# jhidalgocarrio/slam-localization

Measured on NVIDIA B200. Metric: filter-steps/sec (predict+update), higher is better.
Workload: dtype f64

## Files before the change

slam-localization_b200/csrc/slb_usckf_step.cuh:

```cuda
#pragma once
#include "slb_predict12.cuh"

#ifndef SLB_USCKF_CTA_SYNC
#define SLB_USCKF_CTA_SYNC 0
#endif
#if SLB_USCKF_CTA_SYNC
#define SLB_CTA_SYNC() __syncthreads()
#else
#define SLB_CTA_SYNC() ((void)0)
#endif

namespace slbd {

template <int NK_, int NL_>
struct StepCfg {
    static constexpr int NK = NK_, NL = NL_, NF = NK_ + NL_;
    static constexpr int N = 36 + NK_ + NL_;
    static constexpr int NP = N * (N + 1) / 2;
    static constexpr int PSTR = (NP + 15) / 16 * 16;
    static constexpr int QD = 39 + NK_ + NL_;
    static constexpr int QS = (QD + 1) / 2 * 2;
    static constexpr int NT = (N + 7) / 8;
    static constexpr int NPAD = 8 * NT;
    static constexpr int JM = 36 + NK_;
    static constexpr int NPAN = (JM + 3) / 4;
    static constexpr int NCOL = 4 * NPAN;
    static constexpr int JLAST = (NCOL - 1) >> 3;
    static constexpr int NGRP = (NPAN + 3) / 4;
    static constexpr int PL = 2 * NPAD + 8;
    static constexpr int PS4 = 2 * PL + 2;
    static constexpr int KP = (NK_ + 3) / 4 * 4;
    static constexpr int LF = 4 * PS4;
    static constexpr int LRAW = 2 * PL;
    static constexpr int KK = 2 * NPAD * KP + NPAD;
    static constexpr int SCR0 = (LF + LRAW > KK ? LF + LRAW : KK);
    static constexpr int WGS = 16 * NK_;
    static constexpr int UPD_SCR = SCR0 + WGS + NPAD;
    static constexpr int PRED_SCR = PRED_LS + 28 * PRED_DS + 144 + 12 * PRED_DS + 16 + 16;
    static constexpr int SCR = (UPD_SCR > PRED_SCR ? UPD_SCR : PRED_SCR);
    static constexpr int ZS = (NK_ + 1) / 2 * 2;
    static constexpr int SM = PSTR + QS + SCR + ZS + 2;
    static_assert(NK_ % 3 == 0 && NK_ >= 3, "the VO model moves 3-D features");
    static_assert(N <= 64, "two rows per lane");
    static_assert(SM % 2 == 0 && PSTR % 2 == 0 && QS % 2 == 0, "16-byte alignment of the bulk copies");
};

SLB_DEV void bulk_s2g(void *gdst, const void *ssrc, unsigned bytes) {
    asm volatile("cp.async.bulk.global.shared::cta.bulk_group [%0], [%1], %2;\n cp.async.bulk.commit_group;\n" ::"l"(gdst),
                 "r"(saddr(ssrc)), "r"(bytes)
                 : "memory");
}
SLB_DEV void bulk_prefetch_l2(const void *gsrc, unsigned bytes) {
    asm volatile("cp.async.bulk.prefetch.L2.global [%0], %1;\n" ::"l"(gsrc), "r"(bytes) : "memory");
}
SLB_DEV void bulk_store_wait() { asm volatile("cp.async.bulk.wait_group.read 0;\n" ::: "memory"); }
SLB_DEV void fence_proxy_async() { asm volatile("fence.proxy.async.shared::cta;\n" ::: "memory"); }

template <int M>
SLB_DEV bool sym_inverse(const double *S, double *Si) {
    double L[M * (M + 1) / 2], dd[M], rd[M];
    bool ok = true;
#pragma unroll
    for (int k = 0; k < M; ++k) {
        double d = S[tri(k, k)];
#pragma unroll
        for (int p = 0; p < k; ++p) d = fma(-L[tri(k, p)] * L[tri(k, p)], dd[p], d);
        ok = ok && (d > 0.0);
        dd[k] = d;
        rd[k] = rcp_fast(d);
#pragma unroll
        for (int i = k + 1; i < M; ++i) {
            double s = S[tri(i, k)];
#pragma unroll
            for (int p = 0; p < k; ++p) s = fma(-L[tri(i, p)] * L[tri(k, p)], dd[p], s);
            L[tri(i, k)] = s * rd[k];
        }
    }
    double X[M * (M + 1) / 2];
#pragma unroll
    for (int j = 0; j < M; ++j) {
        X[tri(j, j)] = 1.0;
#pragma unroll
        for (int i = j + 1; i < M; ++i) {
            double s = 0.0;
#pragma unroll
            for (int p = j; p < i; ++p) s = fma(-L[tri(i, p)], X[tri(p, j)], s);
            X[tri(i, j)] = s;
        }
    }
#pragma unroll
    for (int i = 0; i < M; ++i)
#pragma unroll
        for (int j = 0; j <= i; ++j) {
            double s = 0.0;
#pragma unroll
            for (int k = i; k < M; ++k) s = fma(X[tri(k, i)] * rd[k], X[tri(k, j)], s);
            Si[tri(i, j)] = s;
        }
    return ok;
}

template <int NK>
SLB_DEV void vo_model(const double *pk, const double *qk, const double *pi, const double *qi, const double *f, double *z) {
    double dq[4];
    quat_cmul(qi, qk, dq);
#pragma unroll
    for (int c = 0; c < NK; c += 3) {
        double rz[3];
        rotmat_apply(dq, f + c, rz);
        z[c] = rz[0] + (pk[0] - pi[0]);
        z[c + 1] = rz[1] + (pk[1] - pi[1]);
        z[c + 2] = rz[2] + (pk[2] - pi[2]);
    }
}

SLB_DEV void warp_sum12(const double *v, double *out, double *slots, int lane) {
    double a[8], b[4], c[2], d1;
    const bool h16 = lane & 16, h8 = lane & 8, h4 = lane & 4, h2 = lane & 2;
#pragma unroll
    for (int i = 0; i < 8; ++i) {
        const double lo = v[i], hi = i < 4 ? v[8 + i] : 0.0;
        const double r = __shfl_xor_sync(FULL, h16 ? lo : hi, 16);
        a[i] = (h16 ? hi : lo) + r;
    }
#pragma unroll
    for (int i = 0; i < 4; ++i) {
        const double r = __shfl_xor_sync(FULL, h8 ? a[i] : a[4 + i], 8);
        b[i] = (h8 ? a[4 + i] : a[i]) + r;
    }
#pragma unroll
    for (int i = 0; i < 2; ++i) {
        const double r = __shfl_xor_sync(FULL, h4 ? b[i] : b[2 + i], 4);
        c[i] = (h4 ? b[2 + i] : b[i]) + r;
    }
    {
        const double r = __shfl_xor_sync(FULL, h2 ? c[0] : c[1], 2);
        d1 = (h2 ? c[1] : c[0]) + r;
    }
    d1 += __shfl_xor_sync(FULL, d1, 1);
    const int idx = (h16 ? 8 : 0) + (h8 ? 4 : 0) + (h4 ? 2 : 0) + (h2 ? 1 : 0);
    __syncwarp();
    if (!(lane & 1)) slots[idx] = d1;
    __syncwarp();
#pragma unroll
    for (int i = 0; i < 6; ++i) {
        const double2 t = *reinterpret_cast<const double2 *>(slots + 2 * i);
        out[2 * i] = t.x;
        out[2 * i + 1] = t.y;
    }
}

template <class C>
struct UpdState {
    double c0[C::NT][C::JLAST + 1], c1[C::NT][C::JLAST + 1];
    double px0[C::NK], px1[C::NK];
    double esum[C::NK], eep[C::NK * (C::NK + 1) / 2];
    double z0[C::NK];
    bool ok;
};

template <class C, int G>
SLB_DEV void sigma_group(UpdState<C> &s, const double *mus_, const double *Lf, double *Wg, const double *dv, int lane) {
    constexpr int NK = C::NK, PS4 = C::PS4;
    double mus[40 + NK];
    {
        const double2 *m2 = reinterpret_cast<const double2 *>(mus_);
#pragma unroll
        for (int e = 0; e < 4; ++e) { const double2 v = m2[e]; mus[2 * e] = v.x; mus[2 * e + 1] = v.y; }
#pragma unroll
        for (int e = 13; e < 17; ++e) { const double2 v = m2[e]; mus[2 * e] = v.x; mus[2 * e + 1] = v.y; }
#pragma unroll
        for (int c = 0; c < NK; ++c) mus[39 + c] = mus_[39 + c];
    }
    constexpr int col0 = 16 * G;
    constexpr int ncols = C::NCOL - col0 < 16 ? C::NCOL - col0 : 16;
    const bool neg = lane & 1, act = (lane >> 1) < ncols;
    const int jl = act ? lane >> 1 : 0;
    const double rs = rsqrt_fast(dv[col0 + jl]);
    const double sgn = act ? (neg ? -rs : rs) : 0.0;
    const double *col = Lf + (jl >> 2) * PS4 + ((jl & 3) >> 1) * C::PL + (jl & 1);
    auto Lc = [&](int r) -> double { return sgn * col[2 * r]; };
    double xpk[3], xqk[4], xpi[3], xqi[4], xf[NK];
    if (col0 <= 5) {
#pragma unroll
        for (int c = 0; c < 3; ++c) xpk[c] = mus[c] + Lc(c);
        const double v[3] = {Lc(3), Lc(4), Lc(5)};
        const double q[4] = {mus[3], mus[4], mus[5], mus[6]};
        double e[4];
        so3_exp(v, 1.0, e);
        quat_mul(q, e, xqk);
    } else {
#pragma unroll
        for (int c = 0; c < 3; ++c) xpk[c] = mus[c];
#pragma unroll
        for (int c = 0; c < 4; ++c) xqk[c] = mus[3 + c];
    }
    if (col0 <= 29) {
#pragma unroll
        for (int c = 0; c < 3; ++c) xpi[c] = mus[26 + c] + Lc(24 + c);
        const double v[3] = {Lc(27), Lc(28), Lc(29)};
        const double q[4] = {mus[29], mus[30], mus[31], mus[32]};
        double e[4];
        so3_exp(v, 1.0, e);
        quat_mul(q, e, xqi);
    } else {
#pragma unroll
        for (int c = 0; c < 3; ++c) xpi[c] = mus[26 + c];
#pragma unroll
        for (int c = 0; c < 4; ++c) xqi[c] = mus[29 + c];
    }
#pragma unroll
    for (int c = 0; c < NK; ++c) xf[c] = mus[39 + c] + Lc(36 + c);
    double z[NK];
    vo_model<NK>(xpk, xqk, xpi, xqi, xf, z);
    double e[NK];
#pragma unroll
    for (int c = 0; c < NK; ++c) {
        e[c] = act ? z[c] - s.z0[c] : 0.0;
        s.esum[c] += e[c];
        const double zp = __shfl_xor_sync(FULL, z[c], 1);
        if (act && !neg) Wg[c * 16 + jl] = (0.5 * rs) * (z[c] - zp);
    }
#pragma unroll
    for (int r = 0; r < NK; ++r)
#pragma unroll
        for (int c = 0; c <= r; ++c) s.eep[tri(r, c)] = fma(e[r], e[c], s.eep[tri(r, c)]);
    __syncwarp();
    const bool has1 = lane + 32 < C::NPAD;
#pragma unroll
    for (int qq = 0; qq < ncols / 4; ++qq) {
        const double *pa = Lf + qq * PS4 + 2 * lane, *pb = pa + C::PL;
        const double2 x01 = *reinterpret_cast<const double2 *>(pa), x23 = *reinterpret_cast<const double2 *>(pb);
        double2 y01 = make_double2(0.0, 0.0), y23 = y01;
        if (has1) { y01 = *reinterpret_cast<const double2 *>(pa + 64); y23 = *reinterpret_cast<const double2 *>(pb + 64); }
#pragma unroll
        for (int c = 0; c < NK; ++c) {
            const double2 w01 = *reinterpret_cast<const double2 *>(Wg + c * 16 + 4 * qq);
            const double2 w23 = *reinterpret_cast<const double2 *>(Wg + c * 16 + 4 * qq + 2);
            s.px0[c] = fma(x23.y, w23.y, fma(x23.x, w23.x, fma(x01.y, w01.y, fma(x01.x, w01.x, s.px0[c]))));
            s.px1[c] = fma(y23.y, w23.y, fma(y23.x, w23.x, fma(y01.y, w01.y, fma(y01.x, w01.x, s.px1[c]))));
        }
    }
}

template <class C, int P>
struct PanelStep {
    SLB_DEV static void run(UpdState<C> &s, const double *mus, double *Lf, double *Lraw, double *Wg, double *dv, int lane) {
        constexpr int NT = C::NT, JLAST = C::JLAST, PS4 = C::PS4;
        constexpr int K = 4 * P, J0 = K >> 3, H = (K >> 2) & 1, Q = P & 3;
        constexpr int I1 = (K + 4) >> 3;
        const int a_ = lane & 3, b_ = lane >> 2;
        double *Lq = Lf + Q * PS4;
        constexpr int PL = C::PL;
        if ((a_ >> 1) == H) {
#pragma unroll
            for (int I = J0; I < NT; ++I)
                *reinterpret_cast<double2 *>(Lraw + (a_ & 1) * PL + 2 * (8 * I + b_)) = make_double2(s.c0[I][J0], s.c1[I][J0]);
        }
        __syncwarp();
        double m10, m20, m30, m21, m31, m32, r0, r1, r2, r3, d0, d1, d2, d3;
        {
            const double *A = Lraw + 2 * K, *Bp = A + PL;
            const double a00 = A[0];
            const double2 a1 = *reinterpret_cast<const double2 *>(A + 2);
            const double2 a2 = *reinterpret_cast<const double2 *>(A + 4);
            const double a22 = Bp[4];
            const double2 a3 = *reinterpret_cast<const double2 *>(A + 6), a3b = *reinterpret_cast<const double2 *>(Bp + 6);
            d0 = a00;
            r0 = rcp_fast(d0);
            m10 = a1.x * r0; m20 = a2.x * r0; m30 = a3.x * r0;
            d1 = fma(-a1.x, m10, a1.y);
            const double u21 = fma(-a2.x, m10, a2.y), u31 = fma(-a3.x, m10, a3.y);
            r1 = rcp_fast(d1);
            m21 = u21 * r1; m31 = u31 * r1;
            d2 = fma(-u21, m21, fma(-a2.x, m20, a22));
            const double u32 = fma(-u31, m21, fma(-a3.x, m20, a3b.x));
            r2 = rcp_fast(d2);
            m32 = u32 * r2;
            d3 = fma(-u32, m32, fma(-u31, m31, fma(-a3.x, m30, a3b.y)));
            r3 = rcp_fast(d3);
            s.ok = s.ok && (d0 > 0.0) && (d1 > 0.0) && (d2 > 0.0) && (d3 > 0.0);
        }
        if (lane == 0) {
            *reinterpret_cast<double2 *>(dv + K) = make_double2(d0, d1);
            *reinterpret_cast<double2 *>(dv + K + 2) = make_double2(d2, d3);
        }
        auto finish = [&](int i, bool have) {
            const double2 x01 = *reinterpret_cast<const double2 *>(Lraw + 2 * i);
            const double2 x23 = *reinterpret_cast<const double2 *>(Lraw + PL + 2 * i);
            const double u0 = x01.x;
            const double u1 = fma(-u0, m10, x01.y);
            const double u2 = fma(-u1, m21, fma(-u0, m20, x23.x));
            const double u3 = fma(-u2, m32, fma(-u1, m31, fma(-u0, m30, x23.y)));
            double2 u01, u23;
            u01.x = i >= K ? u0 : 0.0;
            u01.y = i >= K + 1 ? u1 : 0.0;
            u23.x = i >= K + 2 ? u2 : 0.0;
            u23.y = i >= K + 3 ? u3 : 0.0;
            if (have) {
                *reinterpret_cast<double2 *>(Lq + 2 * i) = u01;
                *reinterpret_cast<double2 *>(Lq + PL + 2 * i) = u23;
            }
        };
        if (K < 32) {
            finish(lane, true);
        } else {
            *reinterpret_cast<double2 *>(Lq + 2 * lane) = make_double2(0.0, 0.0);
            *reinterpret_cast<double2 *>(Lq + PL + 2 * lane) = make_double2(0.0, 0.0);
        }
        if (C::NPAD > 32) finish(lane + 32 < C::NPAD ? lane + 32 : lane, lane + 32 < C::NPAD);
        __syncwarp();
        if (I1 <= JLAST) {
            double f[NT];
            const double *fp = Lq + (a_ >> 1) * PL + (a_ & 1) + 2 * b_;
#pragma unroll
            for (int I = I1; I < NT; ++I) f[I] = fp[16 * I];
            const double rlo = (a_ & 1) ? r1 : r0, rhi = (a_ & 1) ? r3 : r2;
            const double nr = -((a_ & 2) ? rhi : rlo);
#pragma unroll
            for (int J = I1; J <= JLAST; ++J) {
                const double g = f[J] * nr;
#pragma unroll
                for (int I = J; I < NT; ++I) dmma884(s.c0[I][J], s.c1[I][J], f[I], g);
            }
        }
        if (Q == 3 || P == C::NPAN - 1) {
            sigma_group<C, (P >> 2)>(s, mus, Lf, Wg, dv, lane);
            SLB_CTA_SYNC();
        }
        PanelStep<C, P + 1>::run(s, mus, Lf, Lraw, Wg, dv, lane);
    }
};
template <class C>
struct PanelStep<C, C::NPAN> {
    SLB_DEV static void run(UpdState<C> &, const double *, double *, double *, double *, double *, int) {}
};

template <int NK, int NL>
SLB_DEV int usckf_update_smem(double *Ps, double *mus, double *scr, const double *zs, const slb::FilterArgs &a, int lane,
                              bool &dirty) {
    typedef StepCfg<NK, NL> C;
    constexpr int N = C::N, NT = C::NT, NPAD = C::NPAD, JLAST = C::JLAST, KP = C::KP;
    const int a_ = lane & 3, b_ = lane >> 2;
    double *Lf = scr, *Lraw = scr + C::LF, *Ks = scr, *Cs = scr + NPAD * KP, *Wg = scr + C::SCR0, *dv = Wg + C::WGS,
           *dl = Cs + NPAD * KP;
    UpdState<C> s;
    s.ok = true;
    auto elem = [&](int i, int j) -> double {
        if (i >= N || j >= N) return i == j ? 1.0 : 0.0;
        return i >= j ? Ps[prec(N, i, j)] : Ps[prec(N, j, i)];
    };
#pragma unroll
    for (int I = 0; I < NT; ++I)
#pragma unroll
        for (int J = 0; J <= JLAST; ++J)
            if (J < I) {
                double2 v = make_double2(0.0, 0.0);
                if (8 * I + b_ < N) v = *reinterpret_cast<const double2 *>(Ps + prec(N, 8 * I, 8 * J) + 2 * lane);
                s.c0[I][J] = v.x;
                s.c1[I][J] = v.y;
            } else if (J == I) {
                const int i = 8 * I + b_, j = 8 * J + 2 * a_;
                s.c0[I][J] = elem(i, j);
                s.c1[I][J] = elem(i, j + 1);
            }
#pragma unroll
    for (int c = 0; c < NK; ++c) s.px0[c] = s.px1[c] = s.esum[c] = 0.0;
#pragma unroll
    for (int e = 0; e < NK * (NK + 1) / 2; ++e) s.eep[e] = 0.0;
    {
        double pk[3], qk[4], pi[3], qi[4], ft[NK];
#pragma unroll
        for (int c = 0; c < 3; ++c) { pk[c] = mus[c]; pi[c] = mus[26 + c]; }
#pragma unroll
        for (int c = 0; c < 4; ++c) { qk[c] = mus[3 + c]; qi[c] = mus[29 + c]; }
#pragma unroll
        for (int c = 0; c < NK; ++c) ft[c] = mus[39 + c];
        vo_model<NK>(pk, qk, pi, qi, ft, s.z0);
    }
    PanelStep<C, 0>::run(s, mus, Lf, Lraw, Wg, dv, lane);
    if (!s.ok) return SLB_ST_CHOL_FAIL;

    constexpr double NS = (double)(2 * N + 1);
    double ebar[NK], S[NK * (NK + 1) / 2];
    if (NK == 3) {
        double v[12], o[12];
#pragma unroll
        for (int c = 0; c < 3; ++c) v[c] = s.esum[c];
#pragma unroll
        for (int e = 0; e < 6; ++e) v[3 + e] = s.eep[e];
        v[9] = v[10] = v[11] = 0.0;
        warp_sum12(v, o, dv, lane);
#pragma unroll
        for (int c = 0; c < 3; ++c) ebar[c] = o[c] * (1.0 / NS);
#pragma unroll
        for (int r = 0; r < NK; ++r)
#pragma unroll
            for (int c = 0; c <= r; ++c)
                S[tri(r, c)] = 0.5 * fma(-NS * ebar[r], ebar[c], o[3 + tri(r, c)]) + __ldg(a.R + r * NK + c);
    } else {
#pragma unroll
        for (int c = 0; c < NK; ++c) ebar[c] = warp_sum(s.esum[c]) * (1.0 / NS);
#pragma unroll
        for (int r = 0; r < NK; ++r)
#pragma unroll
            for (int c = 0; c <= r; ++c)
                S[tri(r, c)] = 0.5 * fma(-NS * ebar[r], ebar[c], warp_sum(s.eep[tri(r, c)])) + __ldg(a.R + r * NK + c);
    }
    double Si[NK * (NK + 1) / 2];
    const bool sok = sym_inverse<NK>(S, Si);
    auto SiAt = [&](int r, int c) { return r >= c ? Si[tri(r, c)] : Si[tri(c, r)]; };
    asm volatile("cp.async.wait_group 0;\n" ::: "memory");
    __syncwarp();
    double nu[NK], sn[NK], m2 = 0.0;
#pragma unroll
    for (int c = 0; c < NK; ++c) nu[c] = zs[c] - (s.z0[c] + ebar[c]);
#pragma unroll
    for (int r = 0; r < NK; ++r) {
        double t = 0.0;
#pragma unroll
        for (int c = 0; c < NK; ++c) t = fma(SiAt(r, c), nu[c], t);
        sn[r] = t;
        m2 = fma(nu[r], t, m2);
    }
    if (!sok) return SLB_ST_CHOL_FAIL;
    if (!chi2_accept(m2, a.gate)) return SLB_ST_GATE_REJECT;
    auto finish_row = [&](const double *px, int i) {
        double dsum = 0.0;
#pragma unroll
        for (int c = 0; c < KP; ++c) {
            double k = 0.0;
            if (c < NK) {
#pragma unroll
                for (int p = 0; p < NK; ++p) k = fma(px[p], SiAt(p, c), k);
                dsum = fma(px[c], sn[c], dsum);
            }
            Ks[i * KP + c] = k;
            Cs[i * KP + c] = c < NK ? -px[c] : 0.0;
        }
        dl[i] = dsum;
    };
    finish_row(s.px0, lane);
    if (lane + 32 < NPAD) finish_row(s.px1, lane + 32);
    __syncwarp();
    dirty = true;
    bool finite = true;
    if (lane < 12) {
        const int mbw = lane & 3;
        const int mqo = 13 * (lane >> 2) + (mbw == 0 ? 0 : mbw == 1 ? 3 : mbw == 2 ? 7 : 10);
        const double v[3] = {dl[3 * lane], dl[3 * lane + 1], dl[3 * lane + 2]};
        if (mbw == 1) {
            const double q[4] = {mus[mqo], mus[mqo + 1], mus[mqo + 2], mus[mqo + 3]};
            double e[4], o[4];
            so3_exp(v, 1.0, e);
            quat_mul(q, e, o);
#pragma unroll
            for (int c = 0; c < 4; ++c) { mus[mqo + c] = o[c]; finite = finite && isfinite(o[c]); }
        } else {
#pragma unroll
            for (int c = 0; c < 3; ++c) {
                const double o = mus[mqo + c] + v[c];
                mus[mqo + c] = o;
                finite = finite && isfinite(o);
            }
        }
    }
    for (int f = lane; f < NK + NL; f += 32) {
        const double o = mus[39 + f] + dl[36 + f];
        mus[39 + f] = o;
        finite = finite && isfinite(o);
    }
    {
        double fa[NT][KP / 4], fb[NT][KP / 4];
#pragma unroll
        for (int I = 0; I < NT; ++I)
#pragma unroll
            for (int kk = 0; kk < KP / 4; ++kk) {
                fa[I][kk] = Cs[(8 * I + b_) * KP + 4 * kk + a_];
                fb[I][kk] = Ks[(8 * I + b_) * KP + 4 * kk + a_];
            }
#pragma unroll
        for (int I = 0; I < NT; ++I)
#pragma unroll
            for (int J = 0; J <= I; ++J) {
                const int i = 8 * I + b_, j = 8 * J + 2 * a_;
                if (J < I) {
                    double2 *pp = reinterpret_cast<double2 *>(Ps + prec(N, 8 * I, 8 * J) + 2 * lane);
                    const bool w = i < N;
                    double2 p = w ? *pp : make_double2(0.0, 0.0);
#pragma unroll
                    for (int kk = 0; kk < KP / 4; ++kk) dmma884(p.x, p.y, fa[I][kk], fb[J][kk]);
                    if (w) *pp = p;
                } else {
                    const bool w0 = i < N && j <= i, w1 = i < N && j + 1 <= i;
                    double p0 = w0 ? Ps[prec(N, i, j)] : 0.0, p1 = w1 ? Ps[prec(N, i, j + 1)] : 0.0;
#pragma unroll
                    for (int kk = 0; kk < KP / 4; ++kk) dmma884(p0, p1, fa[I][kk], fb[J][kk]);
                    if (w0) Ps[prec(N, i, j)] = p0;
                    if (w1) Ps[prec(N, i, j + 1)] = p1;
                }
            }
    }
    return __all_sync(FULL, finite) ? 0 : SLB_ST_NONFINITE;
}

template <int PM, int NF>
SLB_DEV int usckf_predict_smem(double *Ps, double *mus, double *scr, const double *u, double dt, const double *Qg, int lane,
                               bool &dirty) {
    typedef LayState12 L;
    typedef CycCfg<12> C;
    constexpr int ROW0 = 24, MU0 = 26, N = 36 + NF;
    double *Ls = scr, *D = Ls + PRED_LS, *W = D + 28 * PRED_DS, *Fk = W + 144, *rsd = Fk + 12 * PRED_DS, *slots = rsd + 16;
    auto PR = [&](int r, int c) -> double & { return Ps[prec(N, ROW0 + r, c)]; };
    auto PF = [&](int fr, int c) -> double & { return Ps[prec(N, 36 + fr, 24 + c)]; };
    const int a_ = lane & 3, b_ = lane >> 2;
    double mu[13];
#pragma unroll
    for (int c = 0; c < 13; ++c) mu[c] = mus[MU0 + c];
    ProcessModel<PM> f;
    f.prepare(u, dt);
    double T[C::RT][C::CT];
#pragma unroll
    for (int r = 0; r < C::RT; ++r)
#pragma unroll
        for (int c = 0; c < C::CT; ++c)
            if (C::exists(r, c)) {
                const int i = a_ + 4 * r, j = b_ + 8 * c;
                T[r][c] = (i < 12 && j <= i) ? PR(i, ROW0 + j) : 0.0;
            }
    bool ok = true;
    {
        const double x0 = __shfl_sync(FULL, T[0][0], 0);
        CholStep<C, 0>::run(T, Ls, a_, b_, ok, x0, -rcp_fast(x0));
    }
    if (!ok) return SLB_ST_CHOL_FAIL;
    __syncwarp();
    if (lane < 12) {
        double sq_, rs_;
        sqrt_rsqrt(Ls[C::cb(lane)], sq_, rs_);
        rsd[lane] = rs_;
    }
    __syncwarp();
    const bool act = lane < 25;
    const int j = lane >= 1 ? (lane - 1) >> 1 : 0, jc = j < 12 ? j : 11;
    double Y[13];
    {
        const double sgn = (lane & 1) ? rsd[jc] : -rsd[jc];
        const int cj = C::cb(jc) - jc;
        double d[12], X[13];
#pragma unroll
        for (int r = 0; r < 12; ++r) d[r] = (act && lane >= 1 && r >= jc) ? sgn * Ls[cj + r] : 0.0;
        boxplus<L>(mu, d, 1.0, X);
        f.apply(X, Y);
    }
    double ref[13];
#pragma unroll
    for (int c = 0; c < 13; ++c) ref[c] = bcast(Y[c], 0);
    int it = 0;
    double nrm2;
    do {
        double dd[12], md[12], nr[13];
        boxminus<L>(Y, ref, dd);
#pragma unroll
        for (int r = 0; r < 12; ++r) dd[r] = act ? dd[r] : 0.0;
        warp_sum12(dd, md, slots, lane);
        nrm2 = 0.0;
#pragma unroll
        for (int r = 0; r < 12; ++r) {
            md[r] *= (1.0 / 25.0);
            nrm2 += md[r] * md[r];
        }
        boxplus<L>(ref, md, 1.0, nr);
#pragma unroll
        for (int c = 0; c < 13; ++c) ref[c] = nr[c];
    } while (sqrt(nrm2) > 1e-6 && ++it < 10000);
    int st = (it >= 10000) ? SLB_ST_MEAN_NOCONV : 0;
    {
        double dY[12];
        boxminus<L>(Y, ref, dY);
        if (lane < 28) {
#pragma unroll
            for (int r = 0; r < 12; r += 2)
                *reinterpret_cast<double2 *>(D + lane * PRED_DS + r) = act ? make_double2(dY[r], dY[r + 1]) : make_double2(0.0, 0.0);
        }
    }
    __syncwarp();
    dirty = true;
    {
        double c00[2] = {0.0, 0.0}, c10[2] = {0.0, 0.0}, c11[2] = {0.0, 0.0};
        const double *p0 = D + a_ * PRED_DS + b_, *p1 = p0 + 8;
#pragma unroll
        for (int k0 = 0; k0 < 28; k0 += 4) {
            const double f0 = p0[k0 * PRED_DS], f1 = p1[k0 * PRED_DS];
            dmma884(c00[0], c00[1], f0, f0);
            dmma884(c10[0], c10[1], f1, f0);
            dmma884(c11[0], c11[1], f1, f1);
        }
        for (int e = lane; e < 144; e += 32) {
            const int jj = e / 12, c = e - jj * 12;
            W[e] = 0.5 * (D[(1 + 2 * jj) * PRED_DS + c] - D[(2 + 2 * jj) * PRED_DS + c]);
        }
        __syncwarp();
        auto put = [&](int r, int c, double v) {
            if (r < 12 && c <= r) PR(r, ROW0 + c) = 0.5 * v + __ldg(Qg + r * 12 + c);
        };
        const int r = b_, c = 2 * a_;
        put(r, c, c00[0]); put(r, c + 1, c00[1]);
        put(8 + r, c, c10[0]); put(8 + r, c + 1, c10[1]);
        put(8 + r, 8 + c, c11[0]); put(8 + r, 8 + c + 1, c11[1]);
    }
    if (lane < 12) {
        double x[12];
#pragma unroll
        for (int r = 11; r >= 0; --r) {
            double sacc = 0.0;
#pragma unroll
            for (int p = r + 1; p < 12; ++p) sacc = fma(Ls[C::cb(r) - r + p], x[p], sacc);
            const double rs = rsd[r];
            x[r] = (W[r * 12 + lane] - rs * sacc) * rs;
        }
#pragma unroll
        for (int r = 0; r < 12; ++r) Fk[lane * PRED_DS + r] = x[r];
    }
    __syncwarp();
    double oc[2][3][2];
    {
        const int r0 = min(b_, 11), r1 = min(8 + b_, 11);
#pragma unroll
        for (int I = 0; I < 2; ++I)
#pragma unroll
            for (int J = 0; J < 3; ++J) oc[I][J][0] = oc[I][J][1] = 0.0;
#pragma unroll
        for (int k0 = 0; k0 < 12; k0 += 4) {
            const double fa0 = Fk[r0 * PRED_DS + k0 + a_], fa1 = Fk[r1 * PRED_DS + k0 + a_];
#pragma unroll
            for (int J = 0; J < 3; ++J) {
                const double bv = PR(k0 + a_, 8 * J + b_);
                dmma884(oc[0][J][0], oc[0][J][1], fa0, bv);
                dmma884(oc[1][J][0], oc[1][J][1], fa1, bv);
            }
        }
    }
    constexpr int NFT = (NF + 7) / 8;
    double of[NFT > 0 ? NFT : 1][2][2];
    {
        const int c0 = min(b_, 11), c1 = min(8 + b_, 11);
#pragma unroll
        for (int I = 0; I < NFT; ++I) {
            of[I][0][0] = of[I][0][1] = of[I][1][0] = of[I][1][1] = 0.0;
            const int fr = min(8 * I + b_, NF - 1);
#pragma unroll
            for (int k0 = 0; k0 < 12; k0 += 4) {
                const double av = PF(fr, k0 + a_);
                dmma884(of[I][0][0], of[I][0][1], av, Fk[c0 * PRED_DS + k0 + a_]);
                dmma884(of[I][1][0], of[I][1][1], av, Fk[c1 * PRED_DS + k0 + a_]);
            }
        }
    }
    __syncwarp();
#pragma unroll
    for (int I = 0; I < 2; ++I)
#pragma unroll
        for (int J = 0; J < 3; ++J)
            if (8 * I + b_ < 12)
                *reinterpret_cast<double2 *>(Ps + prec(N, ROW0 + 8 * I, 8 * J) + 2 * lane) = make_double2(oc[I][J][0], oc[I][J][1]);
#pragma unroll
    for (int I = 0; I < NFT; ++I) {
#pragma unroll
        for (int J = 0; J < 2; ++J) {
            const int fr = 8 * I + b_, c = 8 * J + 2 * a_;
            if (fr < NF && c < 12) { PF(fr, c) = of[I][J][0]; PF(fr, c + 1) = of[I][J][1]; }
        }
    }
    bool finite = true;
#pragma unroll
    for (int c = 0; c < 13; ++c) {
        finite = finite && isfinite(ref[c]);
        if (lane == c) mus[MU0 + c] = ref[c];
    }
    if (!finite) st |= SLB_ST_NONFINITE;
    __syncwarp();
    return st;
}

template <int PM, int NK, int NL, bool PRED, bool UPD, int WPB, int MINB>
__global__ void __launch_bounds__(WPB * 32, MINB) usckf_step_kernel(slb::FilterArgs a) {
    typedef StepCfg<NK, NL> C;
    extern __shared__ __align__(128) double smem[];
    const int lane = threadIdx.x & 31, w = threadIdx.x >> 5;
    const int inst = blockIdx.x * WPB + w;
    if (inst >= a.B) return;
    double *Ps = smem + (size_t)w * C::SM, *mus = Ps + C::PSTR, *scr = mus + C::QS, *zs = scr + C::SCR;
    uint64_t *bar = reinterpret_cast<uint64_t *>(zs + C::ZS);
    double *Pg = a.P + (size_t)inst * a.pstride;
    double *mug = a.mu + (size_t)inst * a.qstride;
    if (lane == 0) {
        mbar_init(bar, 1);
        mbar_expect_tx(bar, (C::PSTR + C::QS) * 8);
        bulk_g2s(Ps, Pg, C::PSTR * 8, bar);
        bulk_g2s(mus, mug, C::QS * 8, bar);
        if (a.prefetch > 0 && inst + a.prefetch < a.B) bulk_prefetch_l2(Pg + (size_t)a.prefetch * a.pstride, C::PSTR * 8);
    }
    if (UPD && lane < NK) {
        asm volatile("cp.async.ca.shared.global [%0], [%1], 8;\n cp.async.commit_group;\n" ::"r"(saddr(zs + lane)),
                     "l"(a.z + (size_t)inst * NK + lane)
                     : "memory");
    }
    double u[ProcessModel<PM>::NU];
    if (PRED) {
#pragma unroll
        for (int c = 0; c < ProcessModel<PM>::NU; ++c) u[c] = a.u[(size_t)inst * ProcessModel<PM>::NU + c];
    }
    __syncwarp();
    mbar_wait(bar, 0);
    SLB_CTA_SYNC();
    int st = 0;
    bool dirty = false;
    if (PRED) st |= usckf_predict_smem<PM, NK + NL>(Ps, mus, scr, u, a.dt, a.Q, lane, dirty);
    if (PRED) SLB_CTA_SYNC();
    if (UPD) st |= usckf_update_smem<NK, NL>(Ps, mus, scr, zs, a, lane, dirty);
    asm volatile("cp.async.wait_group 0;\n" ::: "memory");
    if (dirty) {
        fence_proxy_async();
        __syncwarp();
        if (lane == 0) bulk_s2g(Pg, Ps, C::PSTR * 8);
        for (int e = lane; e < C::QD; e += 32) mug[e] = mus[e];
    }
    if (a.mu_out) {
        __syncwarp();
        for (int e = lane; e < a.out_len; e += 32) a.mu_out[(size_t)inst * a.out_len + e] = mus[a.out_off + e];
    }
    if (st && lane == 0) a.status[inst] |= st;
    if (dirty && lane == 0) bulk_store_wait();
}

}
```

Baseline: 97.41 million.

## Compute cross-covariance accumulation with FP64 DMMA tiles instead of scalar FMAs

The per-sigma-group accumulation of the state/measurement cross-covariance moves from per-lane scalar FMA chains over Wg to 8x8x4 double-precision tensor-core MMAs on fragment-layout accumulators. The Wg stride is padded to 20, and the Cholesky panel finish now only writes the live rows below the panel. Column reads in the sigma builder mask the upper-triangle entries, since those rows are no longer zeroed. The result tiles are spilled to shared memory before the gain computation. This trades scalar FMA throughput for DMMA plus extra masking and a shared-memory round trip.

```diff
diff --git a/slam-localization_b200/csrc/slb_usckf_step.cuh b/slam-localization_b200/csrc/slb_usckf_step.cuh
--- a/slam-localization_b200/csrc/slb_usckf_step.cuh
+++ b/slam-localization_b200/csrc/slb_usckf_step.cuh
@@ -30,11 +30,13 @@
     static constexpr int PL = 2 * NPAD + 8;
     static constexpr int PS4 = 2 * PL + 2;
     static constexpr int KP = (NK_ + 3) / 4 * 4;
+    static constexpr int NTN = (NK_ + 7) / 8;
     static constexpr int LF = 4 * PS4;
     static constexpr int LRAW = 2 * PL;
     static constexpr int KK = 2 * NPAD * KP + NPAD;
     static constexpr int SCR0 = (LF + LRAW > KK ? LF + LRAW : KK);
-    static constexpr int WGS = 16 * NK_;
+    static constexpr int WS = 20;
+    static constexpr int WGS = WS * NK_;
     static constexpr int UPD_SCR = SCR0 + WGS + NPAD;
     static constexpr int PRED_SCR = PRED_LS + 28 * PRED_DS + 144 + 12 * PRED_DS + 16 + 16;
     static constexpr int SCR = (UPD_SCR > PRED_SCR ? UPD_SCR : PRED_SCR);
@@ -153,7 +155,7 @@
 template <class C>
 struct UpdState {
     double c0[C::NT][C::JLAST + 1], c1[C::NT][C::JLAST + 1];
-    double px0[C::NK], px1[C::NK];
+    double x0[C::NT][C::NTN], x1[C::NT][C::NTN];
     double esum[C::NK], eep[C::NK * (C::NK + 1) / 2];
     double z0[C::NK];
     bool ok;
@@ -178,8 +180,9 @@
     const int jl = act ? lane >> 1 : 0;
     const double rs = rsqrt_fast(dv[col0 + jl]);
     const double sgn = act ? (neg ? -rs : rs) : 0.0;
+    constexpr int RW = 8 * ((col0 + ncols - 1) >> 3);
     const double *col = Lf + (jl >> 2) * PS4 + ((jl & 3) >> 1) * C::PL + (jl & 1);
-    auto Lc = [&](int r) -> double { return sgn * col[2 * r]; };
+    auto Lc = [&](int r) -> double { return sgn * (r >= RW || r >= col0 + jl ? col[2 * r] : 0.0); };
     double xpk[3], xqk[4], xpi[3], xqi[4], xf[NK];
     if (col0 <= 5) {
 #pragma unroll
@@ -219,26 +222,26 @@
         e[c] = act ? z[c] - s.z0[c] : 0.0;
         s.esum[c] += e[c];
         const double zp = __shfl_xor_sync(FULL, z[c], 1);
-        if (act && !neg) Wg[c * 16 + jl] = (0.5 * rs) * (z[c] - zp);
+        if (act && !neg) Wg[c * C::WS + jl] = (0.5 * rs) * (z[c] - zp);
     }
 #pragma unroll
     for (int r = 0; r < NK; ++r)
 #pragma unroll
         for (int c = 0; c <= r; ++c) s.eep[tri(r, c)] = fma(e[r], e[c], s.eep[tri(r, c)]);
     __syncwarp();
-    const bool has1 = lane + 32 < C::NPAD;
+    const int a_ = lane & 3, b_ = lane >> 2;
 #pragma unroll
     for (int qq = 0; qq < ncols / 4; ++qq) {
-        const double *pa = Lf + qq * PS4 + 2 * lane, *pb = pa + C::PL;
-        const double2 x01 = *reinterpret_cast<const double2 *>(pa), x23 = *reinterpret_cast<const double2 *>(pb);
-        double2 y01 = make_double2(0.0, 0.0), y23 = y01;
-        if (has1) { y01 = *reinterpret_cast<const double2 *>(pa + 64); y23 = *reinterpret_cast<const double2 *>(pb + 64); }
-#pragma unroll
-        for (int c = 0; c < NK; ++c) {
-            const double2 w01 = *reinterpret_cast<const double2 *>(Wg + c * 16 + 4 * qq);
-            const double2 w23 = *reinterpret_cast<const double2 *>(Wg + c * 16 + 4 * qq + 2);
-            s.px0[c] = fma(x23.y, w23.y, fma(x23.x, w23.x, fma(x01.y, w01.y, fma(x01.x, w01.x, s.px0[c]))));
-            s.px1[c] = fma(y23.y, w23.y, fma(y23.x, w23.x, fma(y01.y, w01.y, fma(y01.x, w01.x, s.px1[c]))));
+        const int J0 = (col0 + 4 * qq) >> 3;
+        const double *fp = Lf + qq * PS4 + (a_ >> 1) * C::PL + (a_ & 1) + 2 * b_;
+        double w[C::NTN];
+#pragma unroll
+        for (int T = 0; T < C::NTN; ++T) w[T] = 8 * T + b_ < NK ? Wg[(8 * T + b_) * C::WS + 4 * qq + a_] : 0.0;
+#pragma unroll
+        for (int I = J0; I < C::NT; ++I) {
+            const double f = fp[16 * I];
+#pragma unroll
+            for (int T = 0; T < C::NTN; ++T) dmma884(s.x0[I][T], s.x1[I][T], f, w[T]);
         }
     }
 }
@@ -285,7 +288,8 @@
             *reinterpret_cast<double2 *>(dv + K) = make_double2(d0, d1);
             *reinterpret_cast<double2 *>(dv + K + 2) = make_double2(d2, d3);
         }
-        auto finish = [&](int i, bool have) {
+        constexpr int R0 = 8 * J0, NLIVE = C::NPAD - R0;
+        auto finish = [&](int i) {
             const double2 x01 = *reinterpret_cast<const double2 *>(Lraw + 2 * i);
             const double2 x23 = *reinterpret_cast<const double2 *>(Lraw + PL + 2 * i);
             const double u0 = x01.x;
@@ -297,18 +301,11 @@
             u01.y = i >= K + 1 ? u1 : 0.0;
             u23.x = i >= K + 2 ? u2 : 0.0;
             u23.y = i >= K + 3 ? u3 : 0.0;
-            if (have) {
-                *reinterpret_cast<double2 *>(Lq + 2 * i) = u01;
-                *reinterpret_cast<double2 *>(Lq + PL + 2 * i) = u23;
-            }
+            *reinterpret_cast<double2 *>(Lq + 2 * i) = u01;
+            *reinterpret_cast<double2 *>(Lq + PL + 2 * i) = u23;
         };
-        if (K < 32) {
-            finish(lane, true);
-        } else {
-            *reinterpret_cast<double2 *>(Lq + 2 * lane) = make_double2(0.0, 0.0);
-            *reinterpret_cast<double2 *>(Lq + PL + 2 * lane) = make_double2(0.0, 0.0);
-        }
-        if (C::NPAD > 32) finish(lane + 32 < C::NPAD ? lane + 32 : lane, lane + 32 < C::NPAD);
+        if (NLIVE >= 32 || lane < NLIVE) finish(R0 + lane);
+        if (NLIVE > 32 && lane < NLIVE - 32) finish(R0 + 32 + lane);
         __syncwarp();
         if (I1 <= JLAST) {
             double f[NT];
@@ -365,7 +362,11 @@
                 s.c1[I][J] = elem(i, j + 1);
             }
 #pragma unroll
-    for (int c = 0; c < NK; ++c) s.px0[c] = s.px1[c] = s.esum[c] = 0.0;
+    for (int I = 0; I < NT; ++I)
+#pragma unroll
+        for (int T = 0; T < C::NTN; ++T) s.x0[I][T] = s.x1[I][T] = 0.0;
+#pragma unroll
+    for (int c = 0; c < NK; ++c) s.esum[c] = 0.0;
 #pragma unroll
     for (int e = 0; e < NK * (NK + 1) / 2; ++e) s.eep[e] = 0.0;
     {
@@ -425,7 +426,17 @@
     }
     if (!sok) return SLB_ST_CHOL_FAIL;
     if (!chi2_accept(m2, a.gate)) return SLB_ST_GATE_REJECT;
-    auto finish_row = [&](const double *px, int i) {
+#pragma unroll
+    for (int I = 0; I < NT; ++I)
+#pragma unroll
+        for (int T = 0; T < C::NTN; ++T)
+            if (8 * T + 2 * a_ < KP)
+                *reinterpret_cast<double2 *>(Cs + (8 * I + b_) * KP + 8 * T + 2 * a_) = make_double2(s.x0[I][T], s.x1[I][T]);
+    __syncwarp();
+    auto finish_row = [&](int i) {
+        double px[NK];
+#pragma unroll
+        for (int c = 0; c < NK; ++c) px[c] = Cs[i * KP + c];
         double dsum = 0.0;
 #pragma unroll
         for (int c = 0; c < KP; ++c) {
@@ -440,8 +451,8 @@
         }
         dl[i] = dsum;
     };
-    finish_row(s.px0, lane);
-    if (lane + 32 < NPAD) finish_row(s.px1, lane + 32);
+    finish_row(lane);
+    if (lane + 32 < NPAD) finish_row(lane + 32);
     __syncwarp();
     dirty = true;
     bool finite = true;
```

Result: faster. 101.5 million (median of 6 runs) (+4.2%).
